# AIflowerQ/InvPref_KDD_2022

Hardware: AMD Instinct MI355X
Metric: training interactions/sec, Yahoo-implicit InvPref (higher is better)
Workload: dtype f32

## Files before the change

### invpref_kdd_2022_amd/csrc/canon_math.hpp

```cpp
#pragma once
#include <hip/hip_runtime.h>

namespace invpref {

__device__ __forceinline__ float bits_to_float(unsigned u) { return __builtin_bit_cast(float, u); }
__device__ __forceinline__ unsigned float_to_bits(float f) { return __builtin_bit_cast(unsigned, f); }

__device__ __forceinline__ float pow2i(int n) { return bits_to_float((unsigned)(n + 127) << 23); }

__device__ __forceinline__ float c_exp(float x) {
    float n = __builtin_rintf(x * 1.44269504f);
    float r = __builtin_fmaf(n, -0.693359375f, x);
    r = __builtin_fmaf(n, 2.12194440e-4f, r);
    float p = 1.9875691500e-4f;
    p = __builtin_fmaf(p, r, 1.3981999507e-3f);
    p = __builtin_fmaf(p, r, 8.3334519073e-3f);
    p = __builtin_fmaf(p, r, 4.1665795894e-2f);
    p = __builtin_fmaf(p, r, 1.6666665459e-1f);
    p = __builtin_fmaf(p, r, 5.0000001201e-1f);
    float r2 = r * r;
    float y = __builtin_fmaf(p, r2, r);
    y = y + 1.0f;
    int ni = (int)n;
    int h = ni >> 1;
    float res = (y * pow2i(h)) * pow2i(ni - h);
    res = (x > 88.72283f) ? __builtin_inff() : res;
    res = (x < -87.33654f) ? 0.0f : res;
    return res;
}

__device__ __forceinline__ float c_log(float x) {
    float xs = x;
    int eadj = 0;
    if (x < 1.17549435e-38f) { xs = x * 8388608.0f; eadj = -23; }
    unsigned u = float_to_bits(xs);
    int e = (int)((u >> 23) & 0xffu) - 126 + eadj;
    float m = bits_to_float((u & 0x007fffffu) | 0x3f000000u);
    if (m < 0.707106781f) { e -= 1; m = (m + m) - 1.0f; } else { m = m - 1.0f; }
    float z = m * m;
    float p = 7.0376836292e-2f;
    p = __builtin_fmaf(p, m, -1.1514610310e-1f);
    p = __builtin_fmaf(p, m, 1.1676998740e-1f);
    p = __builtin_fmaf(p, m, -1.2420140846e-1f);
    p = __builtin_fmaf(p, m, 1.4249322787e-1f);
    p = __builtin_fmaf(p, m, -1.6668057665e-1f);
    p = __builtin_fmaf(p, m, 2.0000714765e-1f);
    p = __builtin_fmaf(p, m, -2.4999993993e-1f);
    p = __builtin_fmaf(p, m, 3.3333331174e-1f);
    float y = (m * z) * p;
    float fe = (float)e;
    y = __builtin_fmaf(fe, -2.12194440e-4f, y);
    y = __builtin_fmaf(-0.5f, z, y);
    float r = m + y;
    r = __builtin_fmaf(fe, 0.693359375f, r);
    r = (x == __builtin_inff()) ? x : r;
    r = (x == 0.0f) ? -__builtin_inff() : r;
    r = (x < 0.0f) ? __builtin_nanf("") : r;
    r = (x != x) ? x : r;
    return r;
}

__device__ __forceinline__ float c_log1p(float x) {
    float u = 1.0f + x;
    float r = c_log(u) * (x / (u - 1.0f));
    return (u == 1.0f) ? x : r;
}

__device__ __forceinline__ float c_sigmoid(float x) { return 1.0f / (1.0f + c_exp(-x)); }

__device__ __forceinline__ float c_bce(float s, float y) {
    float a = c_log1p(-s);
    a = a > -100.0f ? a : -100.0f;
    float b = c_log(s);
    b = b > -100.0f ? b : -100.0f;
    return (y - 1.0f) * a - y * b;
}

__device__ __forceinline__ float c_bce_binary(float s, float y) {
    const float x = -s, u = 1.0f + x;
    const bool one = y == 1.0f;
    float l = c_log(one ? s : u);
    const float l1p = (u == 1.0f) ? x : l * (x / (u - 1.0f));
    l = one ? l : l1p;
    l = l > -100.0f ? l : -100.0f;
    return -l;
}

__device__ __forceinline__ float c_dbce(float s, float y) {
    float d = (1.0f - s) * s;
    d = d > 1e-12f ? d : 1e-12f;
    return (s - y) / d;
}

__device__ __forceinline__ float c_sign(float x) { return (float)((x > 0.0f) - (x < 0.0f)); }

__device__ __forceinline__ float f_rcp(float x) { return __builtin_amdgcn_rcpf(x); }
__device__ __forceinline__ float f_exp(float x) { return __builtin_amdgcn_exp2f(x * 1.44269504f); }
__device__ __forceinline__ float f_log(float x) { return __builtin_amdgcn_logf(x) * 0.693147181f; }
__device__ __forceinline__ float f_sigmoid(float x) { return f_rcp(1.0f + f_exp(-x)); }
__device__ __forceinline__ float f_bce(float s, float y) {
    float a = f_log(1.0f - s);
    a = a > -100.0f ? a : -100.0f;
    float b = f_log(s);
    b = b > -100.0f ? b : -100.0f;
    return (y - 1.0f) * a - y * b;
}
__device__ __forceinline__ float f_bce_binary(float s, float y) {
    float l = f_log(y == 1.0f ? s : 1.0f - s);
    l = l > -100.0f ? l : -100.0f;
    return -l;
}
__device__ __forceinline__ float f_dbce(float s, float y) {
    float d = (1.0f - s) * s;
    d = d > 1e-12f ? d : 1e-12f;
    return (s - y) * f_rcp(d);
}

template <int CTRL>
__device__ __forceinline__ float dpp_move(float v) {
    return __builtin_bit_cast(float, __builtin_amdgcn_update_dpp(0, __builtin_bit_cast(int, v), CTRL, 0xF, 0xF, true));
}
__device__ __forceinline__ float row16_sum(float x) {
    x = x + dpp_move<0xB1>(x);
    x = x + dpp_move<0x4E>(x);
    x = x + dpp_move<0x141>(x);
    x = x + dpp_move<0x140>(x);
    return x;
}
__device__ __forceinline__ float row16_min(float x) {
    x = __builtin_fminf(x, dpp_move<0xB1>(x));
    x = __builtin_fminf(x, dpp_move<0x4E>(x));
    x = __builtin_fminf(x, dpp_move<0x141>(x));
    x = __builtin_fminf(x, dpp_move<0x140>(x));
    return x;
}
__device__ __forceinline__ float row16_max(float x) {
    x = __builtin_fmaxf(x, dpp_move<0xB1>(x));
    x = __builtin_fmaxf(x, dpp_move<0x4E>(x));
    x = __builtin_fmaxf(x, dpp_move<0x141>(x));
    x = __builtin_fmaxf(x, dpp_move<0x140>(x));
    return x;
}

}
```

### invpref_kdd_2022_amd/csrc/invpref_kernels.hip

```cpp
#include "adam_apply.hpp"
#include "launch.hpp"

using namespace invpref;

namespace {

template <int NC, bool VEC, int EMAX>
__global__ __launch_bounds__(256) void forward_kernel(DevTables t, const int64_t *__restrict__ users,
                                                      const int64_t *__restrict__ items,
                                                      const int64_t *__restrict__ envs, int64_t B, uint32_t flags,
                                                      float *__restrict__ inv, float *__restrict__ envaware,
                                                      float *__restrict__ envout) {
    extern __shared__ __attribute__((aligned(16))) float lds[];
    constexpr int DP = NC * 64;
    float *sEv = lds, *sW = lds + t.E * DP, *sb = sW + t.E * DP;
    stage_table(sEv, t.Ev, t.E, t.D, DP);
    stage_table(sW, t.W, t.E, t.D, DP);
    for (int i = threadIdx.x; i < t.E; i += blockDim.x) sb[i] = t.b[i];
    __syncthreads();
    const int l16 = threadIdx.x & 15;
    const int64_t rows_per_block = blockDim.x / kRow;
    const bool implicit = flags & INVPREF_IMPLICIT;
    for (int64_t s = blockIdx.x * rows_per_block + (threadIdx.x >> 4); s < B; s += gridDim.x * rows_per_block) {
        const int64_t u = users[s], v = items[s];
// ... 352 lines not shown
                }
                float *dst = (isW ? g.W : g.Ev) + e * t.D + d;
                *dst += add;
            }
        } else if (idx < 2 * EDP + EMAX) {
            const int e = idx - 2 * EDP;
            if (e < t.E && !no_grad) {
                float add = (float)v;
                if (dense) { const float bv = t.b[e]; add += 2.f * l2 / (float)t.E * bv + l1 / (float)t.E * c_sign(bv); }
                g.b[e] += add;
            }
        } else {
            sloss[idx - 2 * EDP - EMAX] = v;
        }
    }
    __syncthreads();
    if (last_block && losses6) {
        if (dense && threadIdx.x < 64) {
            double w2 = 0, w1 = 0, b2 = 0, b1 = 0;
            for (int i = threadIdx.x; i < t.E * t.D; i += 64) { const double x = t.W[i]; w2 += x * x; w1 += fabs(x); }
            for (int i = threadIdx.x; i < t.E; i += 64) { const double x = t.b[i]; b2 += x * x; b1 += fabs(x); }
            double r2v = w2 / ((double)t.D * t.E) + b2 / (double)t.E, r1v = w1 / ((double)t.D * t.E) + b1 / (double)t.E;
            for (int m = 32; m >= 1; m >>= 1) { r2v += __shfl_xor(r2v, m, 64); r1v += __shfl_xor(r1v, m, 64); }
            if (threadIdx.x == 0) { sreg[0] = r2v; sreg[1] = r1v; }
        }
        __syncthreads();
        if (threadIdx.x == 0) {
            const double Bn = (double)Bnorm, BD2 = Bn * (double)t.D * 2.0;
            const double Li = sloss[0] / Bn, Le = sloss[1] / Bn, Lc = sloss[2] / Bn;
            const double L2 = sloss[3] / BD2 + sreg[0], L1 = sloss[4] / BD2 + sreg[1];
            losses6[0] += (float)Li; losses6[1] += (float)Le; losses6[2] += (float)Lc;
            losses6[3] += (float)L2; losses6[4] += (float)L1;
            losses6[5] += (float)((double)k.ca * Li + (double)k.cb * Le + (double)k.cc * Lc + (double)l2 * L2 + (double)l1 * L1);
        }
    }
}

__global__ __launch_bounds__(256) void adam_kernel(float *__restrict__ p, float *__restrict__ g, float *__restrict__ m,
                                                   float *__restrict__ v, int64_t n, AdamScalars a, int zero_grad,
                                                   int64_t head) {
    const int64_t tid = blockIdx.x * (int64_t)blockDim.x + threadIdx.x, nthr = (int64_t)gridDim.x * blockDim.x;
    if (head >= 4) {
        for (int64_t i = tid; i < n; i += nthr) adam_scalar_at(p, g, m, v, i, a, zero_grad);
        return;
    }
    const int64_t n4 = (n - head) >> 2;
    float4 *p4 = reinterpret_cast<float4 *>(p + head), *g4 = reinterpret_cast<float4 *>(g + head);
    float4 *m4 = reinterpret_cast<float4 *>(m + head), *v4 = reinterpret_cast<float4 *>(v + head);
    for (int64_t i = tid; i < n4; i += nthr) {
        float4 pp = p4[i], gg = g4[i], mm = m4[i], vv = v4[i];
        adam1(pp.x, gg.x, mm.x, vv.x, a); adam1(pp.y, gg.y, mm.y, vv.y, a);
        adam1(pp.z, gg.z, mm.z, vv.z, a); adam1(pp.w, gg.w, mm.w, vv.w, a);
        p4[i] = pp; m4[i] = mm; v4[i] = vv;
        if (zero_grad) g4[i] = f4zero();
    }
    if (blockIdx.x == 0) {
        if ((int64_t)threadIdx.x < head) adam_scalar_at(p, g, m, v, threadIdx.x, a, zero_grad);
        const int64_t t0 = head + (n4 << 2);
        if (threadIdx.x >= 4 && t0 + (threadIdx.x - 4) < n && threadIdx.x < 8)
            adam_scalar_at(p, g, m, v, t0 + (threadIdx.x - 4), a, zero_grad);
    }
}

struct AdamRanges {
    int64_t off4[4], end4[4];
    int n;
};
__global__ __launch_bounds__(256) void adam_ranges_kernel(float *__restrict__ p, float *__restrict__ g, float *__restrict__ m,
                                                          float *__restrict__ v, AdamRanges r, AdamScalars a, int zero_grad,
                                                          int *sched_state, const SchedRow *sched_table, int sched_n,
                                                          int sched_slot) {
    if (sched_state) a = sched_last_launch(sched_state, sched_table, sched_n, sched_slot);
    const int64_t total = r.end4[r.n - 1];
    for (int64_t j = blockIdx.x * (int64_t)blockDim.x + threadIdx.x; j < total; j += (int64_t)gridDim.x * blockDim.x) {
        int q = 0;
        while (j >= r.end4[q]) q++;
        const int64_t i = r.off4[q] + (j - (q ? r.end4[q - 1] : 0));
        adam_f4_at(p, g, m, v, i, a, zero_grad);
    }
}

constexpr int kEpsTableMaxE = 7;
struct EpsBase { float v[INVPREF_MAX_ENVS]; };
struct Factorials { unsigned long long f[INVPREF_MAX_ENVS + 1]; };
__device__ __forceinline__ unsigned long long unrank_packed(unsigned long long r, int E, const Factorials &fac) {
    unsigned avail = (1u << E) - 1u;
    unsigned long long out = 0;
#pragma unroll
    for (int pos = 0; pos < INVPREF_MAX_ENVS; pos++) {
        if (pos < E) {
            unsigned long long f = 1;
#pragma unroll
            for (int k = 0; k < INVPREF_MAX_ENVS; k++) f = (k == E - 1 - pos) ? fac.f[k] : f;
            const unsigned d = (unsigned)(r / f);
            r -= (unsigned long long)d * f;
            unsigned seen = 0, pick = 0;
#pragma unroll
            for (int b = 0; b < INVPREF_MAX_ENVS; b++) {
                const bool on = (avail >> b) & 1u;
                pick = (on && seen == d) ? (unsigned)b : pick;
                seen += on ? 1u : 0u;
            }
            avail &= ~(1u << pick);
            out |= (unsigned long long)pick << (4 * pos);
        }
    }
    return out;
}
__device__ __forceinline__ unsigned unrank_packed_small(unsigned r, int E) {
    unsigned c[8];
    c[0] = 0;
#pragma unroll
    for (int k = 1; k < 8; k++) { c[k] = r % (unsigned)(k + 1); r /= (unsigned)(k + 1); }
    unsigned avail = (1u << E) - 1u, out = 0;
#pragma unroll
    for (int pos = 0; pos < kEpsTableMaxE; pos++) {
        if (pos < E) {
            unsigned d = 0;
#pragma unroll
            for (int k = 0; k < 8; k++) d = (k == E - 1 - pos) ? c[k] : d;
            unsigned seen = 0, pick = 0;
#pragma unroll
            for (int b = 0; b < 8; b++) {
                const bool on = (avail >> b) & 1u;
                pick = (on && seen == d) ? (unsigned)b : pick;
                seen += on ? 1u : 0u;
            }
            avail &= ~(1u << pick);
            out |= pick << (4 * pos);
        }
    }
    return out;
}
template <typename IT>
__global__ __launch_bounds__(256) void eps_unrank_kernel(const IT *__restrict__ idx, int64_t N, int E, Factorials fac,
                                                         unsigned long long *__restrict__ packed) {
    for (int64_t s = blockIdx.x * (int64_t)blockDim.x + threadIdx.x; s < N; s += (int64_t)gridDim.x * blockDim.x)
        packed[s] = unrank_packed(min((unsigned long long)idx[s], fac.f[E] - 1ull), E, fac);
}
constexpr int kTicketShards = 32;
struct EstepFin {
    int *state;
    int64_t *ring;
    int ring_cap;
    int64_t *counts;
    int64_t *diff;
    float *class_w;
    const unsigned *perm_table;
};
__device__ __forceinline__ int ld_sc1_i(const int *p) { return __hip_atomic_load(p, __ATOMIC_RELAXED, __HIP_MEMORY_SCOPE_AGENT); }
__device__ __forceinline__ void st_sc1_i(int *p, int v) { __hip_atomic_store(p, v, __ATOMIC_RELAXED, __HIP_MEMORY_SCOPE_AGENT); }

constexpr int kEstepNumSgpr = 80;
template <int NC, bool VEC, bool NARROW>
__global__ __launch_bounds__(256) __attribute__((amdgpu_num_sgpr(kEstepNumSgpr))) void estep_assign_kernel(DevTables t, const int64_t *__restrict__ users,
                                                           const int64_t *__restrict__ items,
                                                           const float *__restrict__ scores, int64_t N, uint32_t flags,
                                                           const float *__restrict__ eps_rows,
                                                           const unsigned long long *__restrict__ eps_packed, EpsBase eps_base,
                                                           const void *__restrict__ eps_index, int eps_index_bytes,
                                                           int eps_rows_n, Factorials fac,
                                                           const int64_t *old_envs, int64_t *new_envs,
                                                           int *slabs, EstepFin fin) {
    extern __shared__ __attribute__((aligned(16))) float lds[];
    constexpr int DP = NC * 64;
    float *sEv = lds;
    int *cnt = reinterpret_cast<int *>(lds + t.E * DP);
    float *sbase = lds + t.E * DP + INVPREF_MAX_ENVS + 1;
    stage_table(sEv, t.Ev, t.E, t.D, DP);
    for (int i = threadIdx.x; i <= t.E; i += blockDim.x) cnt[i] = 0;
    unsigned *stab = reinterpret_cast<unsigned *>(sbase + INVPREF_MAX_ENVS);
    if (eps_packed || eps_index) {
#pragma unroll
        for (int k = 0; k < INVPREF_MAX_ENVS; k++)
            if (threadIdx.x == k) sbase[k] = eps_base.v[k];
    }
    const int64_t rows_per_block = blockDim.x / kRow;
    const int64_t chunk = ((N + gridDim.x - 1) / gridDim.x + rows_per_block - 1) / rows_per_block * rows_per_block;
    const int64_t s_begin = blockIdx.x * chunk, s_end = min(N, s_begin + chunk);
    auto load_idx = [&](int64_t sx) -> unsigned {
        return eps_index_bytes == 1 ? (unsigned)reinterpret_cast<const uint8_t *>(eps_index)[sx]
                                    : (unsigned)reinterpret_cast<const int32_t *>(eps_index)[sx];
    };
    if (eps_index) {
        if (fin.perm_table)
            for (int i = threadIdx.x; i < eps_rows_n; i += blockDim.x) stab[i] = fin.perm_table[i];
        else
            for (int i = threadIdx.x; i < eps_rows_n; i += blockDim.x) stab[i] = unrank_packed_small((unsigned)i, t.E);
    }
    __syncthreads();
    const int l16 = threadIdx.x & 15;
    const bool implicit = flags & INVPREF_IMPLICIT;
    float eps_thr = 0.f;
    if (eps_packed || eps_index) {
        float mx = 0.f;
#pragma unroll
        for (int k = 0; k < INVPREF_MAX_ENVS; k++) mx = (k < t.E) ? __builtin_fmaxf(mx, __builtin_fabsf(eps_base.v[k])) : mx;
        eps_thr = mx * 67108864.f * 1.001f;
    }
    const int64_t s_first = s_begin + (threadIdx.x >> 4);
    const bool idx_bulk = eps_index && eps_index_bytes == 1;
    const int lane64 = threadIdx.x & 63, grp_w = lane64 >> 4;
    auto load_bulk = [&](int blk) -> unsigned {
        const int64_t sx = s_begin + ((threadIdx.x >> 6) * 4 + (lane64 & 3)) + rows_per_block * ((int64_t)blk * 16 + (lane64 >> 2));
        return sx < s_end ? (unsigned)reinterpret_cast<const uint8_t *>(eps_index)[sx] : 0u;
    };
    unsigned bulk_cur = idx_bulk ? load_bulk(0) : 0u, bulk_next = 0u;
    unsigned idx_cur = (eps_index && !idx_bulk && s_first < s_end) ? load_idx(s_first) : 0u;
    int pass = 0;
    for (int64_t s = s_first; s < s_end; s += rows_per_block, pass++) {
        unsigned idx_next = 0u;
        if (idx_bulk) {
            const int pk = __builtin_amdgcn_readfirstlane(pass);
            if ((pk & 15) == 0) {
                if (pk) bulk_cur = bulk_next;
                bulk_next = load_bulk((pk >> 4) + 1);
            }
            const int src = (pk & 15) * 4;
            const unsigned i0 = __builtin_amdgcn_readlane(bulk_cur, src), i1 = __builtin_amdgcn_readlane(bulk_cur, src + 1);
            const unsigned i2 = __builtin_amdgcn_readlane(bulk_cur, src + 2), i3 = __builtin_amdgcn_readlane(bulk_cur, src + 3);
            idx_cur = grp_w == 0 ? i0 : (grp_w == 1 ? i1 : (grp_w == 2 ? i2 : i3));
        } else if (eps_index && s + rows_per_block < s_end) {
            idx_next = load_idx(s + rows_per_block);
        }
        const int64_t u = users[s], v = items[s];
        const float y = scores[s];
        float4 pu[NC], qi[NC], pa[NC], qa[NC];
        if (NARROW) {
            const unsigned uo = (unsigned)u * (unsigned)t.D, vo = (unsigned)v * (unsigned)t.D;
            load_row<NC, VEC>(t.Pu + uo, 0, t.D, l16, pu);
            load_row<NC, VEC>(t.Qi + vo, 0, t.D, l16, qi);
            load_row<NC, VEC>(t.Pa + uo, 0, t.D, l16, pa);
            load_row<NC, VEC>(t.Qa + vo, 0, t.D, l16, qa);
        } else {
            load_row<NC, VEC>(t.Pu, u, t.D, l16, pu);
            load_row<NC, VEC>(t.Qi, v, t.D, l16, qi);
            load_row<NC, VEC>(t.Pa, u, t.D, l16, pa);
            load_row<NC, VEC>(t.Qa, v, t.D, l16, qa);
        }
        const float p = dot2<NC>(pu, qi);
        const float sp = implicit ? c_sigmoid(p) : p;
        float qmine = 0.f;
        for (int c = 0; c < t.E; c++) {
            float4 ev[NC];
            lds_row<NC>(sEv, c, l16, ev);
            const float q = dot3<NC>(pa, qa, ev);
            qmine = (l16 == c) ? q : qmine;
        }
        float dist;
        if (implicit) {
            const float sv = sp * c_sigmoid(qmine);
            const bool binary = __builtin_amdgcn_ballot_w64(!(y == 0.0f || y == 1.0f)) == 0;
            dist = binary ? c_bce_binary(sv, y) : c_bce(sv, y);
        } else { const float r = (p + qmine) - y; dist = r * r; }
        if (eps_rows && l16 < t.E) dist = dist + eps_rows[s * t.E + l16];
        if (eps_packed || eps_index) {
            const bool need = row16_min(l16 < t.E ? dist : __builtin_inff()) < eps_thr;
            if (need) {
                if (eps_packed && l16 < t.E) dist = dist + sbase[(eps_packed[s] >> (4 * l16)) & 15ull];
                if (eps_index && l16 < t.E)
                    dist = dist + sbase[(stab[min(idx_cur, (unsigned)(eps_rows_n - 1))] >> (4 * l16)) & 15u];
            }
        }
        dist = l16 < t.E ? dist : __builtin_inff();
        const float dmin = row16_min(dist);
        const int bi_num = (int)row16_min(dist == dmin ? (float)l16 : 99.f);
        const int bi_nan = (int)row16_min(dist != dist ? (float)l16 : 99.f);
        const int bi = bi_nan < 99 ? bi_nan : bi_num;
        if (l16 == 0) {
            const int64_t was = old_envs ? old_envs[s] : (int64_t)bi;
            const bool changed = was != (int64_t)bi;
            new_envs[s] = bi;
            atomicAdd(cnt + bi, 1);
            if (changed) atomicAdd(cnt + t.E, 1);
        }
        if (!idx_bulk) idx_cur = idx_next;
    }
    __syncthreads();
    if (!fin.state) {
        for (int i = threadIdx.x; i <= t.E; i += blockDim.x) slabs[(int64_t)blockIdx.x * (t.E + 1) + i] = cnt[i];
        return;
    }
    __shared__ int s_last;
    __shared__ long long s_tot[INVPREF_MAX_ENVS + 1];
    if (threadIdx.x < 64) {
        if ((int)threadIdx.x <= t.E) {
            const int S0 = min(kTicketShards, (int)gridDim.x);
            __hip_atomic_fetch_add(fin.state + 32 + 32 * ((int)blockIdx.x % S0) + 1 + (int)threadIdx.x, cnt[threadIdx.x], __ATOMIC_RELAXED,
                                   __HIP_MEMORY_SCOPE_AGENT);
        }
        asm volatile("s_waitcnt vmcnt(0)" ::: "memory");
        if (threadIdx.x == 0) {
            const int S = min(kTicketShards, (int)gridDim.x), sh = (int)blockIdx.x % S;
            const int members = ((int)gridDim.x - sh + S - 1) / S;
            int *tk = fin.state + 32 + 32 * sh;
            int last = 0;
            if (__hip_atomic_fetch_add(tk, 1, __ATOMIC_RELAXED, __HIP_MEMORY_SCOPE_AGENT) == members - 1) {
                st_sc1_i(tk, 0);
                last = __hip_atomic_fetch_add(fin.state, 1, __ATOMIC_RELAXED, __HIP_MEMORY_SCOPE_AGENT) == S - 1;
            }
            s_last = last;
        }
    }
    for (int i = threadIdx.x; i <= t.E; i += blockDim.x) s_tot[i] = 0;
    __syncthreads();
    if (!s_last) return;
    {
        const int E1 = t.E + 1, nsl = (int)gridDim.x;
        const int S0 = min(kTicketShards, nsl);
        for (int i = threadIdx.x; i < S0 * E1; i += blockDim.x) {
            int *w = fin.state + 32 + 32 * (i / E1) + 1 + i % E1;
            const int x = ld_sc1_i(w);
            st_sc1_i(w, 0);
            atomicAdd((unsigned long long *)&s_tot[i % E1], (unsigned long long)(long long)x);
        }
        __syncthreads();
        int64_t *row = nullptr;
        if (fin.ring) row = fin.ring + (int64_t)((unsigned)fin.state[1] % (unsigned)fin.ring_cap) * E1;
        if ((int)threadIdx.x < t.E) {
            const long long c = s_tot[threadIdx.x];
            const long long r = (c + 1 < N - 1) ? c + 1 : N - 1;
            if (fin.counts) fin.counts[threadIdx.x] = c;
            if (fin.class_w) fin.class_w[threadIdx.x] = (float)((double)r / (double)N);
            if (row) row[threadIdx.x] = c;
        }
        if (threadIdx.x == 0) {
            if (fin.diff) *fin.diff = s_tot[t.E];
            if (row) row[t.E] = s_tot[t.E];
        }
        __syncthreads();
        if (threadIdx.x == 0) {
            if (fin.ring) fin.state[1] = fin.state[1] + 1;
            st_sc1_i(fin.state, 0);
        }
    }
}

__global__ __launch_bounds__(256) void env_hist_kernel(const int64_t *__restrict__ envs, int64_t N, int E,
                                                       int *__restrict__ slabs) {
    __shared__ int cnt[INVPREF_MAX_ENVS + 1];
    for (int i = threadIdx.x; i <= E; i += blockDim.x) cnt[i] = 0;
    __syncthreads();
    for (int64_t s = blockIdx.x * (int64_t)blockDim.x + threadIdx.x; s < N; s += (int64_t)gridDim.x * blockDim.x)
        atomicAdd(cnt + (int)envs[s], 1);
    __syncthreads();
    for (int i = threadIdx.x; i <= E; i += blockDim.x) slabs[(int64_t)blockIdx.x * (E + 1) + i] = cnt[i];
}

__global__ __launch_bounds__(256) void stat_envs_kernel(const int64_t *__restrict__ envs, int64_t N, int E,
                                                        const int *__restrict__ slabs, int nslabs,
                                                        int64_t *__restrict__ counts, int64_t *__restrict__ diff,
                                                        float *__restrict__ class_w, float *__restrict__ sample_w) {
    __shared__ long long tot[INVPREF_MAX_ENVS + 1];
    __shared__ float cw[INVPREF_MAX_ENVS];
    for (int i = threadIdx.x; i <= E; i += blockDim.x) tot[i] = 0;
    __syncthreads();
    long long acc[INVPREF_MAX_ENVS + 1];
#pragma unroll
    for (int c = 0; c <= INVPREF_MAX_ENVS; c++) acc[c] = 0;
    for (int s = threadIdx.x; s < nslabs; s += blockDim.x) {
        const int *row = slabs + (int64_t)s * (E + 1);
#pragma unroll
        for (int c = 0; c <= INVPREF_MAX_ENVS; c++) acc[c] += (c <= E) ? row[min(c, E)] : 0;
    }
#pragma unroll
    for (int c = 0; c <= INVPREF_MAX_ENVS; c++) {
        if (c <= E) {
            long long a = acc[c];
            for (int m = 32; m >= 1; m >>= 1) a += __shfl_xor(a, m, 64);
            if ((threadIdx.x & 63) == 0) atomicAdd((unsigned long long *)&tot[c], (unsigned long long)a);
        }
    }
    __syncthreads();
    if (threadIdx.x < E) {
        const long long c = tot[threadIdx.x];
        const long long r = (c + 1 < N - 1) ? c + 1 : N - 1;
        const float w = (float)((double)r / (double)N);
        cw[threadIdx.x] = w;
        if (blockIdx.x == 0) {
            counts[threadIdx.x] = c;
            if (class_w) class_w[threadIdx.x] = w;
        }
    }
    if (blockIdx.x == 0 && threadIdx.x == 0 && diff) *diff = tot[E];
    __syncthreads();
    if (sample_w) {
        const int64_t stride = (int64_t)gridDim.x * blockDim.x * 4;
        for (int64_t s0 = (blockIdx.x * (int64_t)blockDim.x + threadIdx.x) * 4; s0 < N; s0 += stride) {
            int e[4];
#pragma unroll
            for (int k = 0; k < 4; k++) e[k] = (int)envs[min(s0 + k, N - 1)];
#pragma unroll
            for (int k = 0; k < 4; k++)
                if (s0 + k < N) sample_w[s0 + k] = cw[e[k]];
        }
    }
}

template <int NC, bool VEC>
__global__ __launch_bounds__(256) void predict_kernel(const float *__restrict__ Pu, const float *__restrict__ Qi,
                                                      const int64_t *__restrict__ users, int64_t n, int I, int D,
                                                      int apply_sigmoid, float *__restrict__ out, int per_slice) {
    const int l16 = threadIdx.x & 15;
    const int64_t row = blockIdx.x * (int64_t)(blockDim.x / kRow) + (threadIdx.x >> 4);
    if (row >= n) return;
    float4 pu[NC];
    load_row<NC, VEC>(Pu, users[row], D, l16, pu);
    float *o = out + row * (int64_t)I;
    const int i_lo = blockIdx.y * per_slice;
    int i_hi = i_lo + per_slice;
    i_hi = i_hi < I ? i_hi : I;
    for (int i0 = i_lo; i0 < i_hi; i0 += 16) {
        float res = 0.f;
#pragma unroll 4
        for (int j = 0; j < 16; j++) {
            const int i = i0 + j;
            if (i < i_hi) {
                float4 qi[NC];
                load_row<NC, VEC>(Qi, i, D, l16, qi);
                float p = dot2<NC>(pu, qi);
                if (apply_sigmoid) p = c_sigmoid(p);
                res = (j == l16) ? p : res;
            }
        }
        if (i0 + l16 < i_hi) o[i0 + l16] = res;
    }
}

typedef float f32x4_t __attribute__((ext_vector_type(4)));
// ... 340 lines not shown
    hipLaunchKernelGGL(adam_kernel, dim3((unsigned)nb), dim3(256), 0, (hipStream_t)stream, param, grad, exp_avg,
                       exp_avg_sq, n, a, zero_grad, head);
    return (int)hipGetLastError();
}

int invpref_pack_rows_hip(const float *flat, const int64_t *row_offsets, int64_t n_rows, int32_t D, int64_t tail_offset,
                          int64_t tail_len, float *packed, int vec_ok, void *stream) {
    return pack_rows_launch(false, const_cast<float *>(flat), row_offsets, n_rows, D, tail_offset, tail_len, packed, vec_ok,
                            stream);
}

int invpref_unpack_rows_hip(float *flat, const int64_t *row_offsets, int64_t n_rows, int32_t D, int64_t tail_offset,
                            int64_t tail_len, const float *packed, int vec_ok, void *stream) {
    return pack_rows_launch(true, flat, row_offsets, n_rows, D, tail_offset, tail_len, const_cast<float *>(packed), vec_ok,
                            stream);
}

static int adam_ranges_launch(float *param, float *grad, float *exp_avg, float *exp_avg_sq, const int64_t *offsets,
                              const int64_t *lengths, int32_t n_ranges, const AdamScalars &a, int zero_grad,
                              const InvPrefAdamSchedule *sched, void *stream) {
    if (!param || !grad || !exp_avg || !exp_avg_sq || !offsets || !lengths || n_ranges < 1 || n_ranges > 4)
        return INVPREF_EINVAL;
    if ((reinterpret_cast<uintptr_t>(param) | reinterpret_cast<uintptr_t>(grad) | reinterpret_cast<uintptr_t>(exp_avg) |
         reinterpret_cast<uintptr_t>(exp_avg_sq)) & 15u)
        return INVPREF_EINVAL;
    if (sched && (!sched->state || !sched->table || sched->n <= 0)) return INVPREF_EINVAL;
    AdamRanges r{};
    int64_t total = 0;
    for (int i = 0; i < n_ranges; i++) {
        if (offsets[i] < 0 || lengths[i] <= 0 || (offsets[i] & 3) || (lengths[i] & 3)) return INVPREF_EINVAL;
        r.off4[i] = offsets[i] >> 2;
        total += lengths[i] >> 2;
        r.end4[i] = total;
    }
    r.n = n_ranges;
    int64_t nb = (total + 255) / 256;
    if (nb > 2048) nb = 2048;
    hipLaunchKernelGGL(adam_ranges_kernel, dim3((unsigned)nb), dim3(256), 0, (hipStream_t)stream, param, grad, exp_avg,
                       exp_avg_sq, r, a, zero_grad, sched ? sched->state : nullptr,
                       sched ? reinterpret_cast<const SchedRow *>(sched->table) : nullptr, sched ? sched->n : 0,
                       sched ? (sched->slot & 1) : 0);
    return (int)hipGetLastError();
}

int invpref_adam_ranges_hip(float *param, float *grad, float *exp_avg, float *exp_avg_sq, const int64_t *offsets,
                            const int64_t *lengths, int32_t n_ranges, int64_t step, double lr, double beta1, double beta2,
                            double eps, int zero_grad, void *stream) {
    if (step < 1) return INVPREF_EINVAL;
    return adam_ranges_launch(param, grad, exp_avg, exp_avg_sq, offsets, lengths, n_ranges,
                              adam_scalars(step, lr, beta1, beta2, eps), zero_grad, nullptr, stream);
}

int invpref_adam_ranges_sched_hip(float *param, float *grad, float *exp_avg, float *exp_avg_sq, const int64_t *offsets,
                                  const int64_t *lengths, int32_t n_ranges, const InvPrefAdamSchedule *sched,
                                  int zero_grad, void *stream) {
    if (!sched) return INVPREF_EINVAL;
    return adam_ranges_launch(param, grad, exp_avg, exp_avg_sq, offsets, lengths, n_ranges, AdamScalars{}, zero_grad,
                              sched, stream);
}

size_t invpref_estep_workspace_bytes(const InvPrefTables *tables, int64_t N) {
    const int64_t E = tables ? tables->env_num : INVPREF_MAX_ENVS;
    return sizeof(int) * (size_t)(E + 1) * kEstepMaxBlocks + sizeof(unsigned long long) * (size_t)(N > 0 ? N : 0);
}

int invpref_stat_envs_hip(const int64_t *envs, int64_t N, int64_t env_num, int64_t *counts, float *class_weights,
                          float *sample_weights, void *workspace, size_t workspace_bytes, void *stream) {
    if (!envs || !counts || !workspace || N <= 0 || env_num <= 0) return INVPREF_EINVAL;
    if (env_num > INVPREF_MAX_ENVS) return INVPREF_EUNSUPPORTED;
    if (workspace_bytes < sizeof(int) * (size_t)(env_num + 1) * kEstepMaxBlocks) return INVPREF_EWORKSPACE;
    int64_t nb = (N + 255) / 256;
    if (nb > kEstepMaxBlocks) nb = kEstepMaxBlocks;
    hipStream_t st = (hipStream_t)stream;
    int *slabs = (int *)workspace;
    hipLaunchKernelGGL(env_hist_kernel, dim3((unsigned)nb), dim3(256), 0, st, envs, N, (int)env_num, slabs);
    hipLaunchKernelGGL(stat_envs_kernel, dim3((unsigned)nb), dim3(256), 0, st, envs, N, (int)env_num, slabs, (int)nb,
                       counts, (int64_t *)nullptr, class_weights, sample_weights);
    return (int)hipGetLastError();
}

int invpref_sample_weights_hip(const int64_t *envs, int64_t N_local, const int64_t *counts, int64_t N_total,
                               int64_t env_num, float *class_weights, float *sample_weights, void *stream) {
    if (!counts || N_local < 0 || N_total <= 0 || env_num <= 0 || (N_local > 0 && sample_weights && !envs))
        return INVPREF_EINVAL;
    if (env_num > INVPREF_MAX_ENVS) return INVPREF_EUNSUPPORTED;
    int64_t nb = (N_local + 255) / 256;
    if (nb < 1) nb = 1;
    if (nb > kEstepMaxBlocks) nb = kEstepMaxBlocks;
    hipLaunchKernelGGL(sample_weights_kernel, dim3((unsigned)nb), dim3(256), 0, (hipStream_t)stream, envs, N_local, counts,
                       N_total, (int)env_num, class_weights, sample_weights);
    return (int)hipGetLastError();
}

static int estep_launch(const InvPrefTables *tables, const int64_t *users, const int64_t *items, const float *scores,
                        int64_t N, uint32_t flags, const float *eps_rows, const void *perm_index, int index_bytes,
                        const float *eps_base_host, const int64_t *old_envs, int64_t *new_envs, int64_t *counts,
                        int64_t *diff, float *class_weights, float *sample_weights, void *workspace,
                        size_t workspace_bytes, void *stream, const EstepFin *fused = nullptr) {
    int rc = check_tables(tables);
    if (rc) return rc;
    if (N <= 0 || !users || !items || !scores || !new_envs || !workspace) return INVPREF_EINVAL;
    if (!fused && (!counts || !diff)) return INVPREF_EINVAL;
    if (workspace_bytes < invpref_estep_workspace_bytes(tables, N)) return INVPREF_EWORKSPACE;
    const DevTables t = dev_tables(tables);
    const bool vec = vec_ok(tables);
    const int nc = vec ? nc_of(t.D) : 4;
    const int nb = estep_blocks(N);
    const size_t lds = sizeof(float) * ((size_t)t.E * nc * 64 + INVPREF_MAX_ENVS + 1 + INVPREF_MAX_ENVS);
    hipStream_t st = (hipStream_t)stream;
    int *slabs = (int *)workspace;
    unsigned long long *eps_packed = nullptr;
    EpsBase eps_base{};
    Factorials fac{};
    fac.f[0] = 1;
    for (int k = 1; k <= INVPREF_MAX_ENVS; k++) fac.f[k] = fac.f[k - 1] * (unsigned long long)k;
    const void *eps_index = nullptr;
    int eps_rows_n = 0;
    size_t lds_extra = 0;
    if (perm_index) {
        if (eps_rows || !eps_base_host || (index_bytes != 1 && index_bytes != 4 && index_bytes != 8)) return INVPREF_EINVAL;
        if ((index_bytes == 1 && t.E > 5) || (index_bytes == 4 && t.E > 12)) return INVPREF_EINVAL;
        for (int k = 0; k < t.E; k++) eps_base.v[k] = eps_base_host[k];
    }
    bool table_form = perm_index && t.E <= kEpsTableMaxE && index_bytes != 8;
    if (table_form) {
        lds_extra = sizeof(unsigned) * (size_t)fac.f[t.E];
        if (lds + lds_extra > 64 * 1024) { table_form = false; lds_extra = 0; }
    }
    if (table_form) {
        eps_index = perm_index;
        eps_rows_n = (int)fac.f[t.E];
    } else if (perm_index) {
        eps_packed = reinterpret_cast<unsigned long long *>(reinterpret_cast<char *>(workspace) +
                                                           sizeof(int) * (size_t)(t.E + 1) * kEstepMaxBlocks);
        int64_t ub = (N + 255) / 256;
        if (ub > 4096) ub = 4096;
        with_int<1, 4, 8>(index_bytes, [&](auto bytes_c) {
            constexpr int W = decltype(bytes_c)::value;
            using IT = std::conditional_t<W == 1, uint8_t, std::conditional_t<W == 4, int32_t, int64_t>>;
            hipLaunchKernelGGL(eps_unrank_kernel<IT>, dim3((unsigned)ub), dim3(256), 0, st, (const IT *)perm_index, N, t.E, fac,
                               eps_packed);
            return 0;
        });
    }
    EstepFin fin{};
    if (fused) {
        fin = *fused;
        if (!table_form) fin.perm_table = nullptr;
    }
    static const bool force64 = std::getenv("INVPREF_ESTEP_OFFSETS64") != nullptr && std::getenv("INVPREF_ESTEP_OFFSETS64")[0] == '1';
    const bool narrow = !force64 && (uint64_t)std::max(t.U, t.I) * (uint64_t)t.D * 4u < (1ull << 32);
    rc = with_nv(nc, vec, [&](auto nc_c, auto vec_c) {
        return with_bool(narrow, [&](auto narrow_c) {
            hipLaunchKernelGGL((estep_assign_kernel<decltype(nc_c)::value, decltype(vec_c)::value, decltype(narrow_c)::value>),
                               dim3(nb), dim3(kEstepThreads), lds + lds_extra, st, t, users, items, scores, N, flags, eps_rows,
                               eps_packed, eps_base, eps_index, index_bytes, eps_rows_n, fac, old_envs, new_envs, slabs, fin);
            return (int)hipGetLastError();
        });
    });
    if (rc) return rc;
    if (fused) return 0;
    int64_t nb2 = (N + 255) / 256;
    if (nb2 > 256) nb2 = 256;
    hipLaunchKernelGGL(stat_envs_kernel, dim3((unsigned)nb2), dim3(256), 0, st, new_envs, N, t.E, slabs, nb, counts, diff,
                       class_weights, sample_weights);
    return (int)hipGetLastError();
}

int invpref_estep_hip(const InvPrefTables *tables, const int64_t *users, const int64_t *items, const float *scores,
                      int64_t N, uint32_t flags, const float *eps_rows, const int64_t *old_envs, int64_t *new_envs,
                      int64_t *counts, int64_t *diff, float *class_weights, float *sample_weights, void *workspace,
                      size_t workspace_bytes, void *stream) {
    return estep_launch(tables, users, items, scores, N, flags, eps_rows, nullptr, 0, nullptr, old_envs, new_envs, counts,
                        diff, class_weights, sample_weights, workspace, workspace_bytes, stream);
}

int invpref_estep_perm_hip(const InvPrefTables *tables, const int64_t *users, const int64_t *items, const float *scores,
                           int64_t N, uint32_t flags, const void *perm_index, int index_bytes, const float *eps_base,
                           const int64_t *old_envs, int64_t *new_envs, int64_t *counts, int64_t *diff,
                           float *class_weights, float *sample_weights, void *workspace, size_t workspace_bytes,
                           void *stream) {
    if (!perm_index) return INVPREF_EINVAL;
    return estep_launch(tables, users, items, scores, N, flags, nullptr, perm_index, index_bytes, eps_base, old_envs,
                        new_envs, counts, diff, class_weights, sample_weights, workspace, workspace_bytes, stream);
}

int invpref_perm_table_fill(int32_t env_num, uint32_t *host_table) {
    if (!host_table || env_num < 1 || env_num > kEpsTableMaxE) return INVPREF_EINVAL;
    int rows = 1;
    for (int k = 2; k <= env_num; k++) rows *= k;
    for (int r = 0; r < rows; r++) {
        unsigned avail = (1u << env_num) - 1u, out = 0;
        int rem = r, f = rows;
        for (int pos = 0; pos < env_num; pos++) {
            f /= (env_num - pos);
            const int d = rem / f;
            rem -= d * f;
            int seen = 0, pick = 0;
            for (int b = 0; b < env_num; b++)
                if ((avail >> b) & 1u) { if (seen == d) pick = b; seen++; }
            avail &= ~(1u << pick);
            out |= (unsigned)pick << (4 * pos);
        }
        host_table[r] = out;
    }
    return rows;
}

int invpref_estep_fused_hip(const InvPrefTables *tables, const int64_t *users, const int64_t *items, const float *scores,
                            int64_t N, uint32_t flags, const void *perm_index, int index_bytes, const float *eps_base,
                            const uint32_t *perm_table, int64_t *envs, int32_t *state, int64_t *ring, int32_t ring_cap,
                            int64_t *counts, int64_t *diff, float *class_weights, void *workspace, size_t workspace_bytes,
                            void *stream) {
    if (!state || !envs || (ring && ring_cap <= 0)) return INVPREF_EINVAL;
    EstepFin fin{};
    fin.state = state; fin.ring = ring; fin.ring_cap = ring_cap; fin.counts = counts; fin.diff = diff;
    fin.class_w = class_weights; fin.perm_table = perm_table;
    return estep_launch(tables, users, items, scores, N, flags, nullptr, perm_index, perm_index ? index_bytes : 0, eps_base, envs,
                        envs, counts, diff, class_weights, nullptr, workspace, workspace_bytes, stream, &fin);
}

}
```

### invpref_kdd_2022_amd/csrc/kernel_common.hpp

```cpp
#pragma once
#include <hip/hip_runtime.h>
#include <stdint.h>

#include "../../include/invpref_hip.h"
#include "canon_math.hpp"

#define WAVE_LDS_FENCE() asm volatile("s_waitcnt lgkmcnt(0)" ::: "memory")

namespace invpref {

constexpr int kRow = 16;
constexpr int kLossSlots = 8;

struct DevTables {
    const float *Pu, *Qi, *Pa, *Qa, *Ev, *W, *b;
    int U, I, E, D;
};
struct DevGrads {
    float *Pu, *Qi, *Pa, *Qa, *Ev, *W, *b;
};

__device__ __forceinline__ float4 f4zero() { return make_float4(0.f, 0.f, 0.f, 0.f); }
__device__ __forceinline__ float4 f4mul(float4 a, float4 b) { return make_float4(a.x * b.x, a.y * b.y, a.z * b.z, a.w * b.w); }

template <int NC, bool VEC>
__device__ __forceinline__ void load_row(const float *__restrict__ base, int64_t row, int D, int l16, float4 (&r)[NC]) {
    const float *p = base + row * (int64_t)D;
#pragma unroll
    for (int c = 0; c < NC; c++) {
        const int i0 = (l16 + kRow * c) * 4;
        if (VEC) {
            r[c] = (i0 < D) ? *reinterpret_cast<const float4 *>(p + i0) : f4zero();
        } else {
            r[c].x = (i0 + 0 < D) ? p[i0 + 0] : 0.f;
            r[c].y = (i0 + 1 < D) ? p[i0 + 1] : 0.f;
            r[c].z = (i0 + 2 < D) ? p[i0 + 2] : 0.f;
            r[c].w = (i0 + 3 < D) ? p[i0 + 3] : 0.f;
        }
    }
}
template <int NC>
__device__ __forceinline__ void lds_row(const float *tab, int e, int l16, float4 (&r)[NC]) {
#pragma unroll
    for (int c = 0; c < NC; c++) r[c] = *reinterpret_cast<const float4 *>(tab + e * (NC * 64) + (l16 + kRow * c) * 4);
}

template <int NC>
__device__ __forceinline__ float dot2(const float4 (&a)[NC], const float4 (&b)[NC]) {
    float s = 0.f;
#pragma unroll
    for (int c = 0; c < NC; c++) {
        s = __builtin_fmaf(a[c].x, b[c].x, s);
        s = __builtin_fmaf(a[c].y, b[c].y, s);
        s = __builtin_fmaf(a[c].z, b[c].z, s);
        s = __builtin_fmaf(a[c].w, b[c].w, s);
    }
    return row16_sum(s);
}
template <int NC>
__device__ __forceinline__ float dot3(const float4 (&a)[NC], const float4 (&b)[NC], const float4 (&cc)[NC]) {
    float s = 0.f;
#pragma unroll
    for (int c = 0; c < NC; c++) {
        s = __builtin_fmaf(a[c].x * b[c].x, cc[c].x, s);
        s = __builtin_fmaf(a[c].y * b[c].y, cc[c].y, s);
        s = __builtin_fmaf(a[c].z * b[c].z, cc[c].z, s);
        s = __builtin_fmaf(a[c].w * b[c].w, cc[c].w, s);
    }
    return row16_sum(s);
}

__device__ __forceinline__ void stage_table(float *dst, const float *__restrict__ src, int E, int D, int DP) {
    for (int i = threadIdx.x; i < E * DP; i += blockDim.x) {
        const int e = i / DP, d = i - e * DP;
        dst[i] = (src && d < D) ? src[e * D + d] : 0.f;
    }
}

__device__ __forceinline__ float wave_sum(float x) {
#pragma unroll
    for (int m = 32; m >= 1; m >>= 1) x += __shfl_xor(x, m, 64);
    return x;
}
__device__ __forceinline__ double wave_sum_f64(double x) {
#pragma unroll
    for (int m = 32; m >= 1; m >>= 1) x += __shfl_xor(x, m, 64);
    return x;
}



struct StepScalars {
    float ca, cb, cc, alpha, invB, r2, r1;
};

struct AdamScalars {
    float step_size, bc2_sqrt, w1, b2, w2, eps;
};
__device__ __forceinline__ void adam1(float &p, float g, float &m, float &v, const AdamScalars &a) {
    m = m + a.w1 * (g - m);
    v = v * a.b2 + (a.w2 * g) * g;
    const float denom = __builtin_sqrtf(v) / a.bc2_sqrt + a.eps;
    p = p + ((-a.step_size) * m) / denom;
}

__device__ __forceinline__ void adam1f(float &p, float g, float &m, float &v, const AdamScalars &a) {
    m = m + a.w1 * (g - m);
    v = v * a.b2 + (a.w2 * g) * g;
    const float denom = __builtin_amdgcn_sqrtf(v) * __builtin_amdgcn_rcpf(a.bc2_sqrt) + a.eps;
    p = p + ((-a.step_size) * m) * __builtin_amdgcn_rcpf(denom);
}

}
```

Baseline: 531.5 million.

## Batch multiple samples per 16-lane row in E-step with scatter-reduce of env dots

```diff
diff --git a/invpref_kdd_2022_amd/csrc/canon_math.hpp b/invpref_kdd_2022_amd/csrc/canon_math.hpp
--- a/invpref_kdd_2022_amd/csrc/canon_math.hpp
+++ b/invpref_kdd_2022_amd/csrc/canon_math.hpp
@@ -120,6 +120,10 @@
 __device__ __forceinline__ float dpp_move(float v) {
     return __builtin_bit_cast(float, __builtin_amdgcn_update_dpp(0, __builtin_bit_cast(int, v), CTRL, 0xF, 0xF, true));
 }
+template <int CTRL>
+__device__ __forceinline__ unsigned dpp_move_u(unsigned v) {
+    return (unsigned)__builtin_amdgcn_update_dpp(0, (int)v, CTRL, 0xF, 0xF, true);
+}
 __device__ __forceinline__ float row16_sum(float x) {
     x = x + dpp_move<0xB1>(x);
     x = x + dpp_move<0x4E>(x);
@@ -134,6 +138,42 @@
     x = __builtin_fminf(x, dpp_move<0x140>(x));
     return x;
 }
+template <int W>
+__device__ __forceinline__ float sub_min(float x) {
+    static_assert(W == 4 || W == 8 || W == 16, "sub-group width");
+    x = __builtin_fminf(x, dpp_move<0xB1>(x));
+    x = __builtin_fminf(x, dpp_move<0x4E>(x));
+    if constexpr (W >= 8) x = __builtin_fminf(x, dpp_move<0x141>(x));
+    if constexpr (W >= 16) x = __builtin_fminf(x, dpp_move<0x140>(x));
+    return x;
+}
+template <int NV>
+__device__ __forceinline__ int scatter_slot(int l16) {
+    static_assert(NV == 4 || NV == 8, "values per row");
+    const int m = (l16 & 8) ? (l16 ^ 15) : l16;
+    const int g = (m & 4) ? (m ^ 7) : m;
+    return NV == 8 ? (g | (m & 4)) : g;
+}
+template <int NV>
+__device__ __forceinline__ float row16_sum_scatter(const float (&s)[NV], int slot) {
+    static_assert(NV == 4 || NV == 8, "values per row");
+    const bool o0 = slot & 1, o1 = slot & 2;
+    float a[NV / 2], b[NV / 4];
+#pragma unroll
+    for (int j = 0; j < NV / 2; j++) a[j] = (o0 ? s[2 * j + 1] : s[2 * j]) + dpp_move<0xB1>(o0 ? s[2 * j] : s[2 * j + 1]);
+#pragma unroll
+    for (int j = 0; j < NV / 4; j++) b[j] = (o1 ? a[2 * j + 1] : a[2 * j]) + dpp_move<0x4E>(o1 ? a[2 * j] : a[2 * j + 1]);
+    float x;
+    if constexpr (NV == 8) {
+        const bool o2 = slot & 4;
+        x = (o2 ? b[1] : b[0]) + dpp_move<0x141>(o2 ? b[0] : b[1]);
+    } else {
+        x = b[0];
+        x = x + dpp_move<0x141>(x);
+    }
+    x = x + dpp_move<0x140>(x);
+    return x;
+}
 __device__ __forceinline__ float row16_max(float x) {
     x = __builtin_fmaxf(x, dpp_move<0xB1>(x));
     x = __builtin_fmaxf(x, dpp_move<0x4E>(x));
diff --git a/invpref_kdd_2022_amd/csrc/invpref_kernels.hip b/invpref_kdd_2022_amd/csrc/invpref_kernels.hip
--- a/invpref_kdd_2022_amd/csrc/invpref_kernels.hip
+++ b/invpref_kdd_2022_amd/csrc/invpref_kernels.hip
@@ -528,7 +528,8 @@
 __device__ __forceinline__ void st_sc1_i(int *p, int v) { __hip_atomic_store(p, v, __ATOMIC_RELAXED, __HIP_MEMORY_SCOPE_AGENT); }
 
 constexpr int kEstepNumSgpr = 80;
-template <int NC, bool VEC, bool NARROW>
+constexpr int estep_passes(int E) { return E <= 4 ? 4 : (E <= 8 ? 2 : 1); }
+template <int NC, bool VEC, bool NARROW, int PASSES>
 __global__ __launch_bounds__(256) __attribute__((amdgpu_num_sgpr(kEstepNumSgpr))) void estep_assign_kernel(DevTables t, const int64_t *__restrict__ users,
                                                            const int64_t *__restrict__ items,
                                                            const float *__restrict__ scores, int64_t N, uint32_t flags,
@@ -581,76 +582,179 @@
         const int64_t sx = s_begin + ((threadIdx.x >> 6) * 4 + (lane64 & 3)) + rows_per_block * ((int64_t)blk * 16 + (lane64 >> 2));
         return sx < s_end ? (unsigned)reinterpret_cast<const uint8_t *>(eps_index)[sx] : 0u;
     };
-    unsigned bulk_cur = idx_bulk ? load_bulk(0) : 0u, bulk_next = 0u;
-    unsigned idx_cur = (eps_index && !idx_bulk && s_first < s_end) ? load_idx(s_first) : 0u;
-    int pass = 0;
-    for (int64_t s = s_first; s < s_end; s += rows_per_block, pass++) {
-        unsigned idx_next = 0u;
-        if (idx_bulk) {
-            const int pk = __builtin_amdgcn_readfirstlane(pass);
-            if ((pk & 15) == 0) {
-                if (pk) bulk_cur = bulk_next;
-                bulk_next = load_bulk((pk >> 4) + 1);
-            }
-            const int src = (pk & 15) * 4;
-            const unsigned i0 = __builtin_amdgcn_readlane(bulk_cur, src), i1 = __builtin_amdgcn_readlane(bulk_cur, src + 1);
-            const unsigned i2 = __builtin_amdgcn_readlane(bulk_cur, src + 2), i3 = __builtin_amdgcn_readlane(bulk_cur, src + 3);
-            idx_cur = grp_w == 0 ? i0 : (grp_w == 1 ? i1 : (grp_w == 2 ? i2 : i3));
-        } else if (eps_index && s + rows_per_block < s_end) {
-            idx_next = load_idx(s + rows_per_block);
-        }
-        const int64_t u = users[s], v = items[s];
-        const float y = scores[s];
-        float4 pu[NC], qi[NC], pa[NC], qa[NC];
-        if (NARROW) {
-            const unsigned uo = (unsigned)u * (unsigned)t.D, vo = (unsigned)v * (unsigned)t.D;
-            load_row<NC, VEC>(t.Pu + uo, 0, t.D, l16, pu);
-            load_row<NC, VEC>(t.Qi + vo, 0, t.D, l16, qi);
-            load_row<NC, VEC>(t.Pa + uo, 0, t.D, l16, pa);
-            load_row<NC, VEC>(t.Qa + vo, 0, t.D, l16, qa);
-        } else {
-            load_row<NC, VEC>(t.Pu, u, t.D, l16, pu);
-            load_row<NC, VEC>(t.Qi, v, t.D, l16, qi);
-            load_row<NC, VEC>(t.Pa, u, t.D, l16, pa);
-            load_row<NC, VEC>(t.Qa, v, t.D, l16, qa);
-        }
-        const float p = dot2<NC>(pu, qi);
-        const float sp = implicit ? c_sigmoid(p) : p;
-        float qmine = 0.f;
-        for (int c = 0; c < t.E; c++) {
-            float4 ev[NC];
-            lds_row<NC>(sEv, c, l16, ev);
-            const float q = dot3<NC>(pa, qa, ev);
-            qmine = (l16 == c) ? q : qmine;
-        }
-        float dist;
-        if (implicit) {
-            const float sv = sp * c_sigmoid(qmine);
-            const bool binary = __builtin_amdgcn_ballot_w64(!(y == 0.0f || y == 1.0f)) == 0;
-            dist = binary ? c_bce_binary(sv, y) : c_bce(sv, y);
-        } else { const float r = (p + qmine) - y; dist = r * r; }
-        if (eps_rows && l16 < t.E) dist = dist + eps_rows[s * t.E + l16];
-        if (eps_packed || eps_index) {
-            const bool need = row16_min(l16 < t.E ? dist : __builtin_inff()) < eps_thr;
-            if (need) {
-                if (eps_packed && l16 < t.E) dist = dist + sbase[(eps_packed[s] >> (4 * l16)) & 15ull];
-                if (eps_index && l16 < t.E)
-                    dist = dist + sbase[(stab[min(idx_cur, (unsigned)(eps_rows_n - 1))] >> (4 * l16)) & 15u];
-            }
-        }
-        dist = l16 < t.E ? dist : __builtin_inff();
-        const float dmin = row16_min(dist);
-        const int bi_num = (int)row16_min(dist == dmin ? (float)l16 : 99.f);
-        const int bi_nan = (int)row16_min(dist != dist ? (float)l16 : 99.f);
-        const int bi = bi_nan < 99 ? bi_nan : bi_num;
-        if (l16 == 0) {
-            const int64_t was = old_envs ? old_envs[s] : (int64_t)bi;
-            const bool changed = was != (int64_t)bi;
-            new_envs[s] = bi;
-            atomicAdd(cnt + bi, 1);
-            if (changed) atomicAdd(cnt + t.E, 1);
-        }
-        if (!idx_bulk) idx_cur = idx_next;
+    if constexpr (PASSES == 1) {
+        unsigned bulk_cur = idx_bulk ? load_bulk(0) : 0u, bulk_next = 0u;
+        unsigned idx_cur = (eps_index && !idx_bulk && s_first < s_end) ? load_idx(s_first) : 0u;
+        int pass = 0;
+        for (int64_t s = s_first; s < s_end; s += rows_per_block, pass++) {
+            unsigned idx_next = 0u;
+            if (idx_bulk) {
+                const int pk = __builtin_amdgcn_readfirstlane(pass);
+                if ((pk & 15) == 0) {
+                    if (pk) bulk_cur = bulk_next;
+                    bulk_next = load_bulk((pk >> 4) + 1);
+                }
+                const int src = (pk & 15) * 4;
+                const unsigned i0 = __builtin_amdgcn_readlane(bulk_cur, src), i1 = __builtin_amdgcn_readlane(bulk_cur, src + 1);
+                const unsigned i2 = __builtin_amdgcn_readlane(bulk_cur, src + 2), i3 = __builtin_amdgcn_readlane(bulk_cur, src + 3);
+                idx_cur = grp_w == 0 ? i0 : (grp_w == 1 ? i1 : (grp_w == 2 ? i2 : i3));
+            } else if (eps_index && s + rows_per_block < s_end) {
+                idx_next = load_idx(s + rows_per_block);
+            }
+            const int64_t u = users[s], v = items[s];
+            const float y = scores[s];
+            float4 pu[NC], qi[NC], pa[NC], qa[NC];
+            if (NARROW) {
+                const unsigned uo = (unsigned)u * (unsigned)t.D, vo = (unsigned)v * (unsigned)t.D;
+                load_row<NC, VEC>(t.Pu + uo, 0, t.D, l16, pu);
+                load_row<NC, VEC>(t.Qi + vo, 0, t.D, l16, qi);
+                load_row<NC, VEC>(t.Pa + uo, 0, t.D, l16, pa);
+                load_row<NC, VEC>(t.Qa + vo, 0, t.D, l16, qa);
+            } else {
+                load_row<NC, VEC>(t.Pu, u, t.D, l16, pu);
+                load_row<NC, VEC>(t.Qi, v, t.D, l16, qi);
+                load_row<NC, VEC>(t.Pa, u, t.D, l16, pa);
+                load_row<NC, VEC>(t.Qa, v, t.D, l16, qa);
+            }
+            const float p = dot2<NC>(pu, qi);
+            const float sp = implicit ? c_sigmoid(p) : p;
+            float qmine = 0.f;
+            for (int c = 0; c < t.E; c++) {
+                float4 ev[NC];
+                lds_row<NC>(sEv, c, l16, ev);
+                const float q = dot3<NC>(pa, qa, ev);
+                qmine = (l16 == c) ? q : qmine;
+            }
+            float dist;
+            if (implicit) {
+                const float sv = sp * c_sigmoid(qmine);
+                const bool binary = __builtin_amdgcn_ballot_w64(!(y == 0.0f || y == 1.0f)) == 0;
+                dist = binary ? c_bce_binary(sv, y) : c_bce(sv, y);
+            } else { const float r = (p + qmine) - y; dist = r * r; }
+            if (eps_rows && l16 < t.E) dist = dist + eps_rows[s * t.E + l16];
+            if (eps_packed || eps_index) {
+                const bool need = row16_min(l16 < t.E ? dist : __builtin_inff()) < eps_thr;
+                if (need) {
+                    if (eps_packed && l16 < t.E) dist = dist + sbase[(eps_packed[s] >> (4 * l16)) & 15ull];
+                    if (eps_index && l16 < t.E)
+                        dist = dist + sbase[(stab[min(idx_cur, (unsigned)(eps_rows_n - 1))] >> (4 * l16)) & 15u];
+                }
+            }
+            dist = l16 < t.E ? dist : __builtin_inff();
+            const float dmin = row16_min(dist);
+            const int bi_num = (int)row16_min(dist == dmin ? (float)l16 : 99.f);
+            const int bi_nan = (int)row16_min(dist != dist ? (float)l16 : 99.f);
+            const int bi = bi_nan < 99 ? bi_nan : bi_num;
+            if (l16 == 0) {
+                const int64_t was = old_envs ? old_envs[s] : (int64_t)bi;
+                const bool changed = was != (int64_t)bi;
+                new_envs[s] = bi;
+                atomicAdd(cnt + bi, 1);
+                if (changed) atomicAdd(cnt + t.E, 1);
+            }
+            if (!idx_bulk) idx_cur = idx_next;
+        }
+    } else {
+        constexpr int SW = kRow / PASSES;
+        const int sub = l16 / SW, slot = scatter_slot<SW>(l16);
+        const bool slot_ok = slot < t.E;
+        const int64_t super = rows_per_block * PASSES, s_off = (int64_t)sub * rows_per_block;
+        auto pack_bulk = [&](unsigned b) -> unsigned {
+            b <<= 8 * ((lane64 >> 2) & 3);
+            b |= dpp_move_u<0x124>(b);
+            b |= dpp_move_u<0x128>(b);
+            return b;
+        };
+        unsigned bulk_cur = idx_bulk ? pack_bulk(load_bulk(0)) : 0u, bulk_next = 0u;
+        unsigned idx_mine = (eps_index && !idx_bulk && s_first + s_off < s_end) ? load_idx(s_first + s_off) : 0u;
+        int pass = 0;
+        for (int64_t s0 = s_first; s0 < s_end; s0 += super, pass += PASSES) {
+            const int64_t s_mine = s0 + s_off;
+            const bool live = s_mine < s_end;
+            unsigned idx_next = 0u;
+            if (idx_bulk) {
+                const int pk = __builtin_amdgcn_readfirstlane(pass);
+                if ((pk & 15) == 0) {
+                    if (pk) bulk_cur = pack_bulk(bulk_next);
+                    bulk_next = load_bulk((pk >> 4) + 1);
+                }
+                const int src = ((pk & 15) >> 2) * 16;
+                const unsigned i0 = __builtin_amdgcn_readlane(bulk_cur, src), i1 = __builtin_amdgcn_readlane(bulk_cur, src + 1);
+                const unsigned i2 = __builtin_amdgcn_readlane(bulk_cur, src + 2), i3 = __builtin_amdgcn_readlane(bulk_cur, src + 3);
+                const unsigned word = grp_w == 0 ? i0 : (grp_w == 1 ? i1 : (grp_w == 2 ? i2 : i3));
+                idx_mine = (word >> (8 * ((pk & 3) + sub))) & 0xffu;
+            } else if (eps_index && s_mine + super < s_end) {
+                idx_next = load_idx(s_mine + super);
+            }
+            const float y = scores[live ? s_mine : s0];
+            float pmine = 0.f, qmine = 0.f;
+#pragma unroll 1
+            for (int k = 0; k < PASSES; k++) {
+                const int64_t sk = (s0 + k * rows_per_block < s_end) ? s0 + k * rows_per_block : s0;
+                const int64_t u = users[sk], v = items[sk];
+                float4 pu[NC], qi[NC], pa[NC], qa[NC];
+                if constexpr (NARROW && VEC) {
+                    const unsigned uo = (unsigned)u * (unsigned)t.D, vo = (unsigned)v * (unsigned)t.D;
+                    load_row_narrow<NC>(t.Pu, uo, t.D, l16, pu);
+                    load_row_narrow<NC>(t.Qi, vo, t.D, l16, qi);
+                    load_row_narrow<NC>(t.Pa, uo, t.D, l16, pa);
+                    load_row_narrow<NC>(t.Qa, vo, t.D, l16, qa);
+                } else if (NARROW) {
+                    const unsigned uo = (unsigned)u * (unsigned)t.D, vo = (unsigned)v * (unsigned)t.D;
+                    load_row<NC, VEC>(t.Pu + uo, 0, t.D, l16, pu);
+                    load_row<NC, VEC>(t.Qi + vo, 0, t.D, l16, qi);
+                    load_row<NC, VEC>(t.Pa + uo, 0, t.D, l16, pa);
+                    load_row<NC, VEC>(t.Qa + vo, 0, t.D, l16, qa);
+                } else {
+                    load_row<NC, VEC>(t.Pu, u, t.D, l16, pu);
+                    load_row<NC, VEC>(t.Qi, v, t.D, l16, qi);
+                    load_row<NC, VEC>(t.Pa, u, t.D, l16, pa);
+                    load_row<NC, VEC>(t.Qa, v, t.D, l16, qa);
+                }
+                const float p = dot2<NC>(pu, qi);
+                float part[SW];
+#pragma unroll
+                for (int c = 0; c < SW; c++) {
+                    part[c] = 0.f;
+                    if (c < t.E) {
+                        float4 ev[NC];
+                        lds_row<NC>(sEv, c, l16, ev);
+                        part[c] = dot3_lane<NC>(pa, qa, ev);
+                    }
+                }
+                const float q = row16_sum_scatter<SW>(part, slot);
+                pmine = (sub == k) ? p : pmine;
+                qmine = (sub == k) ? q : qmine;
+            }
+            float dist;
+            if (implicit) {
+                const float sv = c_sigmoid(pmine) * c_sigmoid(qmine);
+                const bool binary = __builtin_amdgcn_ballot_w64(!(y == 0.0f || y == 1.0f)) == 0;
+                dist = binary ? c_bce_binary(sv, y) : c_bce(sv, y);
+            } else { const float r = (pmine + qmine) - y; dist = r * r; }
+            const bool mine = slot_ok && live;
+            if (eps_rows && mine) dist = dist + eps_rows[s_mine * t.E + slot];
+            if (eps_packed || eps_index) {
+                const bool need = sub_min<SW>(mine ? dist : __builtin_inff()) < eps_thr;
+                if (need && mine) {
+                    if (eps_packed) dist = dist + sbase[(eps_packed[s_mine] >> (4 * slot)) & 15ull];
+                    if (eps_index) dist = dist + sbase[(stab[min(idx_mine, (unsigned)(eps_rows_n - 1))] >> (4 * slot)) & 15u];
+                }
+            }
+            dist = mine ? dist : __builtin_inff();
+            const float dmin = sub_min<SW>(dist);
+            const int bi_num = (int)sub_min<SW>(dist == dmin ? (float)slot : 99.f);
+            const int bi_nan = (int)sub_min<SW>(dist != dist ? (float)slot : 99.f);
+            const int bi = bi_nan < 99 ? bi_nan : bi_num;
+            if (slot == 0 && live) {
+                const int64_t was = old_envs ? old_envs[s_mine] : (int64_t)bi;
+                const bool changed = was != (int64_t)bi;
+                new_envs[s_mine] = bi;
+                atomicAdd(cnt + bi, 1);
+                if (changed) atomicAdd(cnt + t.E, 1);
+            }
+            if (!idx_bulk) idx_mine = idx_next;
+        }
     }
     __syncthreads();
     if (!fin.state) {
@@ -1297,10 +1401,13 @@
     const bool narrow = !force64 && (uint64_t)std::max(t.U, t.I) * (uint64_t)t.D * 4u < (1ull << 32);
     rc = with_nv(nc, vec, [&](auto nc_c, auto vec_c) {
         return with_bool(narrow, [&](auto narrow_c) {
-            hipLaunchKernelGGL((estep_assign_kernel<decltype(nc_c)::value, decltype(vec_c)::value, decltype(narrow_c)::value>),
-                               dim3(nb), dim3(kEstepThreads), lds + lds_extra, st, t, users, items, scores, N, flags, eps_rows,
-                               eps_packed, eps_base, eps_index, index_bytes, eps_rows_n, fac, old_envs, new_envs, slabs, fin);
-            return (int)hipGetLastError();
+            return with_int<1, 2, 4>(estep_passes(t.E), [&](auto passes_c) {
+                hipLaunchKernelGGL((estep_assign_kernel<decltype(nc_c)::value, decltype(vec_c)::value, decltype(narrow_c)::value,
+                                                        decltype(passes_c)::value>),
+                                   dim3(nb), dim3(kEstepThreads), lds + lds_extra, st, t, users, items, scores, N, flags, eps_rows,
+                                   eps_packed, eps_base, eps_index, index_bytes, eps_rows_n, fac, old_envs, new_envs, slabs, fin);
+                return (int)hipGetLastError();
+            });
         });
     });
     if (rc) return rc;
diff --git a/invpref_kdd_2022_amd/csrc/kernel_common.hpp b/invpref_kdd_2022_amd/csrc/kernel_common.hpp
--- a/invpref_kdd_2022_amd/csrc/kernel_common.hpp
+++ b/invpref_kdd_2022_amd/csrc/kernel_common.hpp
@@ -40,6 +40,15 @@
     }
 }
 template <int NC>
+__device__ __forceinline__ void load_row_narrow(const float *__restrict__ base, unsigned elem, int D, int l16, float4 (&r)[NC]) {
+#pragma unroll
+    for (int c = 0; c < NC; c++) {
+        const int i0 = (l16 + kRow * c) * 4;
+        const unsigned byte = (elem + (unsigned)i0) * 4u;
+        r[c] = (i0 < D) ? *reinterpret_cast<const float4 *>(reinterpret_cast<const char *>(base) + byte) : f4zero();
+    }
+}
+template <int NC>
 __device__ __forceinline__ void lds_row(const float *tab, int e, int l16, float4 (&r)[NC]) {
 #pragma unroll
     for (int c = 0; c < NC; c++) r[c] = *reinterpret_cast<const float4 *>(tab + e * (NC * 64) + (l16 + kRow * c) * 4);
@@ -56,6 +65,18 @@
         s = __builtin_fmaf(a[c].w, b[c].w, s);
     }
     return row16_sum(s);
+}
+template <int NC>
+__device__ __forceinline__ float dot3_lane(const float4 (&a)[NC], const float4 (&b)[NC], const float4 (&cc)[NC]) {
+    float s = 0.f;
+#pragma unroll
+    for (int c = 0; c < NC; c++) {
+        s = __builtin_fmaf(a[c].x * b[c].x, cc[c].x, s);
+        s = __builtin_fmaf(a[c].y * b[c].y, cc[c].y, s);
+        s = __builtin_fmaf(a[c].z * b[c].z, cc[c].z, s);
+        s = __builtin_fmaf(a[c].w * b[c].w, cc[c].w, s);
+    }
+    return s;
 }
 template <int NC>
 __device__ __forceinline__ float dot3(const float4 (&a)[NC], const float4 (&b)[NC], const float4 (&cc)[NC]) {
```

After: 527.6 million. Within noise of the previous version (-0.7%).
